# kieranrcampbell/clonealign

Measured on AMD Instinct MI355X. Metric: ELBO iterations/sec, higher is better.
Workload: dtype f32 variables (contraction: float64 series over gene bins; count-matrix products: int8 MFMA, exact); 1 GPU; synthetic 100000 cells x 5000 genes x 8 clones, K=1, S=1, cell-sharded over 1 GPU(s) (BASELINE.json configs[2]); cells=100000, genes=5000, clones=8, K=1, mc_samples=1, y_storage=u8, y_bytes_per_elem=1, fused_sweep=True, fwd_mfma=True, series_form=True, y_mfma=True, parallelism=single, collective=none, allreduce_doubles_per_train_pass=20764, build_id=cf8e5d62109b05e5

## Files before the change

### clonealign_amd/csrc/ca_eng_create.inc

```

constexpr double CA_ML_STREAM_FIXED_US = 6.6;
constexpr double CA_ML_STREAM_BYTES_PER_US = 5.62e6;
constexpr double CA_ML_MIN_STREAM_US = 45.0;
constexpr int CA_ML_MAX_PER = 4;
struct ca_mom_last_in {
  int slots;
  int n_cu;
  int nb_stream, nb_ovf;
  int ngrp, nred;
  int64_t image_bytes;
};
inline int ca_mom_last_free(const ca_mom_last_in& a) { return std::max(a.slots - a.nb_stream, 0); }
inline int ca_mom_last_free_x(const ca_mom_last_in& a) {
  const int xcd = std::max(a.n_cu / 32, 1);
  return a.slots / xcd - cdiv(a.nb_stream, xcd);
}
inline int ca_mom_last_per(const ca_mom_last_in& a) {
  const int xcd = std::max(a.n_cu / 32, 1), free_x = ca_mom_last_free_x(a);
  if (free_x < 1) return 0;
  return std::max(1, cdiv(a.ngrp, free_x * xcd));
}
inline bool ca_mom_last_pick(const ca_mom_last_in& a) {
  if (a.nb_stream + a.ngrp + a.nred <= a.slots) return false;
  const int per = ca_mom_last_per(a);
// ... 451 lines not shown
    h->mom_free_slots = ca_mom_last_free(ml);
    h->mom_last = variantx_on(h, CA_VARX_MOM_LAST, "CA_MOM_LAST_ON") || (variant_on(h, CA_VAR_MOM_LAST, "CA_MOM_LAST") && ca_mom_last_pick(ml));
    if (h->opt.variant_off & CA_VAR_MOM_LAST) h->mom_last = false;
    if (h->mom_last) {
      const int per = ca_mom_last_per(ml);
      h->mom_per = per < 1 ? CA_MOM_PER : std::min(per, CA_ML_MAX_PER);
      h->mom_nred = 2 * CA_MOM_NRED;
      const int lab = (h->opt.reserved[1] & ~0xFF) ? h->opt.reserved[1] >> 8 : 0;
      if (lab & 15) h->mom_per = lab & 15;
      if (lab & 16) h->mom_nred = CA_MOM_NRED;
      h->mom_ovf_first = (lab & 32) != 0;
    }
  }
  h->cell_lean = h->poly && variant_on(h, CA_VAR_CELL_LEAN, "CA_CELL_LEAN");
  h->cell_mfma = h->poly && variant_on(h, CA_VAR_CELL_MFMA, "CA_CELL_MFMA");
  h->gene_ride = h->poly && variant_on(h, CA_VAR_GENE_RIDE, "CA_GENE_RIDE");
  h->gene_cols = h->gene_ride && (h->opt.reserved[1] == 8 || (h->opt.reserved[1] != 7 && Nn <= CA_GENE_COLS_MAXN));
  h->ride_ok = h->ystore == CA_YSTORE_U8 && K == 1 && D <= 2 && h->fused_ok && !h->c16 && h->fwd_cell && (h->fc_tl == 6 || h->fc_tl == 8 || (h->fc_tl == 2 && h->fc_nbig == 0)) &&
               !h->y_ys && variant_on(h, CA_VAR_Y_RIDE, "CA_Y_RIDE");
  const bool tl1_ok = h->fc_tl == 1 && h->fc_nbig == 0 && !h->c16;
  h->ride_ys = h->y_ys && (!h->ys4 || (h->poly && D == 1 && !h->c16 && !h->s2)) && D <= 2 && h->fused_ok && h->fwd_cell && (h->fc_tl == 6 || tl1_ok || (h->fc_tl == 2 && h->fc_nbig == 0)) &&
               variant_on(h, CA_VAR_Y_RIDE, "CA_Y_RIDE");
  h->yfin_split = h->ride_ys && h->bwd_mfma && h->tail_fuse && variant_on(h, CA_VAR_YFIN_RIDE, "CA_YFIN_RIDE");
  if (h->y_ys && !h->ride_ys) h->async_y = false;
  {
    const int tiles = cdiv(Nn, 16), qb = tiles / std::max(h->n_cu, 1), rb = tiles - qb * h->n_cu;
    h->fwd_bal = h->ride_ys && !h->c16 && !h->s2 && D == 1 && C <= 8 && qb >= 1 && qb <= 6 && h->nk32 >= 96 && h->host_dev && variant_on(h, CA_VAR_FWD_BAL, "CA_FWD_BAL");
    if (h->fwd_bal) {
      h->bal_q = qb; h->bal_r = rb;
      h->bal_nchunk = rb > 0 ? std::min(CA_BAL_MAXCHUNK, h->n_cu / rb) : 0;
// ... 103 lines not shown
```

### clonealign_amd/csrc/ca_eng_loop.inc

```
int wait_y(ca_engine* h, bool all) {
  if (all) {
    if (h->y_pending) HIPCK(h, hipStreamWaitEvent(h->stream, h->ev_ydone, 0));
    h->y_pending = false; h->yw_pending = false;
  } else if (h->yw_pending) {
    HIPCK(h, hipStreamWaitEvent(h->stream, h->ev_ywdone, 0));
    h->yw_pending = false;
  }
  return CA_OK;
}

int make_etamax(ca_engine* h) {
  if (h->D > 0) {
    LAUNCH(h, CA_KERNEL_OTHER, hipLaunchKernelGGL(k_vmm_final, dim3(1), dim3(64), 0, h->stream, h->vmm_part, h->vmm, h->ngblk, h->D));
    LAUNCH(h, CA_KERNEL_OTHER, hipLaunchKernelGGL(k_etamax, dim3(cdiv(h->N, CA_TB)), dim3(CA_TB), 0, h->stream, h->F, h->vmm, h->etamax2, h->N, h->D));
  }
  h->em_stale = false;
  return CA_OK;
}
int ensure_etamax(ca_engine* h) {
  if (!h->em_stale) return CA_OK;
  return make_etamax(h);
}

int refresh_derived(ca_engine* h) {
// ... 758 lines not shown
    if (yfin_rides) { yfin_ride = yfin_args(h, h->ys_nrg, h->ys_nseg); h->yfin_pending = false; }
    if (moments_aside) HIPCK(h, hipStreamWaitEvent(h->stream, h->ev_poly1, 0));
    CACK(prof_begin(h, CA_KERNEL_FWD));
    ca_small_args ltail = no_small_args();
    const bool sh = is_sharded(h) && h->tail_fuse && yfin_rides;
    if (sh) {
      ltail = small_args(h, h->gene_part, 0, 0.f, nullptr, true);
      ltail.ncblk = h->pws.n_cell_blocks;
      if (h->K > 0) { ltail.yw_part = h->yw_part; ltail.n_yw = h->n_yw; }
      ltail.reduce_only = 1; ltail.host_out = nullptr;
    }
    const bool cols_move = yfin_rides && h->gene_cols;
    const bool merges = gene_ride_merges(h);
    ca_yfin_args yfin_cols = yfin_ride;
    if (cols_move) yfin_ride.ncol = 0;
    e = ca_poly_cells(h->stream, &h->pws, h->N, h->C, h->K, &cp, h->alpha_u, h->cell_part, h->dFpart, yfin_rides ? &yfin_ride : nullptr, h->cell_lean, h->cell_mfma);
    h->red_pending = merges;
    if (merges) h->ycol_pending = cols_move;
    else if (e == hipSuccess)
      e = ca_poly_reduce(h->stream, &h->pws, h->N, h->C, cols_move ? &yfin_cols : nullptr, sh ? &ltail : nullptr, h->poly_xmax_ready ? h->poly_xpart : nullptr,
                         (int)cdiv(h->N, CA_TB), h->F, sh ? h->red + h->off_x : nullptr, h->opt.rank, std::max(h->opt.world, 1));
    h->mon_tail_local = sh;
    if (sh) { h->poly_xslot_pending = true; h->poly_xglob_steps = -1; }
    HIPCK(h, e);
    CACK(prof_end(h));
    cell_blocks = h->pws.n_cell_blocks;
    h->poly_fresh = true;
  } else
  if (h->fwd_cell && ride && h->ride_ys) {
    cell_blocks = h->ncblk_f;
    CACK(ys_quant(h));
// ... 201 lines not shown
```

### clonealign_amd/csrc/ca_eng_state.inc

```
namespace {

thread_local std::string g_last_error;

typedef struct { char internal[128]; } ca_nccl_uid;
typedef void* ca_nccl_comm;
struct RcclApi {
  void* lib = nullptr;
  int (*GetUniqueId)(ca_nccl_uid*) = nullptr;
  int (*CommInitRank)(ca_nccl_comm*, int, ca_nccl_uid, int) = nullptr;
  int (*CommDestroy)(ca_nccl_comm) = nullptr;
  int (*AllReduce)(const void*, void*, size_t, int, int, ca_nccl_comm, hipStream_t) = nullptr;
  const char* (*GetErrorString)(int) = nullptr;
  std::string err;
  bool load() {
    if (lib) return true;
    const char* cands[] = {getenv("CLONEALIGN_RCCL_LIB"), "librccl.so.1", "librccl.so", "/opt/rocm/lib/librccl.so.1",
                           "/opt/rocm/lib/librccl.so"};
    for (const char* c : cands) {
      if (!c || !*c) continue;
      lib = dlopen(c, RTLD_NOW | RTLD_LOCAL);
      if (lib) break;
    }
    if (!lib) { err = std::string("cannot dlopen librccl: ") + dlerror(); return false; }
    GetUniqueId = (decltype(GetUniqueId))dlsym(lib, "ncclGetUniqueId");
// ... 103 lines not shown
  bool poly_shape = false, layout_series = false;
  bool mon_tail_local = false;
  bool poly_xslot_pending = false;
  int poly_xglob_steps = -1;
  double* elbo_dev = nullptr; int64_t elbo_cap = 0; double* terms_dev = nullptr;
  double* host_pinned = nullptr;
  bool ycache_valid = false, sums_global = false, sums_started = false;
  std::vector<double> mu_part;
  bool fused_ok = false, look_valid = false; int64_t look_slot = 0; int frow = 8;
  bool carry = false, carry_builtin = false; std::vector<float> carry_eps;
  int64_t n_series = 0, n_series_fallback = 0;
  double *poly_ring = nullptr, *poly_ring_dev = nullptr; uint64_t poly_seq = 0, poly_seq_base = 1, adam_steps = 0, poly_steps_at[16] = {};
  bool mom_ride = false; unsigned mom_tag = 0; const ca_pm_args* mom_args = nullptr;
  bool mom_last = false, mom_ovf_first = false; int mom_free_slots = 0, mom_per = CA_MOM_PER, mom_nred = CA_MOM_NRED;
  bool cell_mfma = false;
  bool cell_lean = false;
  bool gene_cols = false;
  bool gene_ride = false, red_pending = false, ycol_pending = false; unsigned gene_tag = 0; int poly_nb_ub = 0;
  bool poly = false, poly_side = false, poly_y_defer = false, poly_fresh = false, poly_df = false ; ca_poly_ws pws; float* poly_zero = nullptr; unsigned char* poly_mem = nullptr;
  float *Mb2 = nullptr, *mu32B = nullptr, *Zpart2 = nullptr; double* gene_partB = nullptr;
  bool y_defer = false;
  bool ride_ok = false;
  bool ride_ys = false;
  bool fold_gsum = false, fold_now = false;
  int64_t hint_A = -1, hint_B = -1, pre_A = -1, pre_B = -1;
  bool pre_valid = false, pre_ok = true, pair_elbo = true;
  double* ee_partB = nullptr;
  double *gene_part_alt = nullptr, *gene_partB_alt = nullptr;
  bool bwd_ready = false; int64_t bwd_slot = -1;
  double* yw_part = nullptr; int n_yw = 0;
// ... 53 lines not shown
  } while (0)

int comm_check(ca_engine* h) {
  if (h->host_pinned && *reinterpret_cast<volatile unsigned int*>(h->host_pinned + 41) != 0u) {
    h->err = "a forward-sweep block gave up waiting for a chunk of a left-over tile (k_fwd_bal_ys); the engine's state is undefined";
    return CA_ERR_STATE;
  }
  if (h->host_pinned && *reinterpret_cast<volatile unsigned int*>(h->host_pinned + 43) != 0u) {
    h->err = "a reducer block of the series form's moment role gave up waiting for the moment blocks of its launch (k_ys_mfma_mom); the engine's state is undefined";
    return CA_ERR_STATE;
  }
  if (h->host_pinned && *reinterpret_cast<volatile unsigned int*>(h->host_pinned + 44) != 0u) {
    h->err = "a gene block of the series form's merged way back gave up waiting for the reducer blocks of its launch (k_poly_tail); the engine's state is undefined";
    return CA_ERR_STATE;
  }
  if (h->host_pinned && *reinterpret_cast<volatile unsigned int*>(h->host_pinned + 42) != 0u) {
    h->err = "the series form of the contraction (CA_VARX_SERIES) cannot cover this fit's exponent range: max|psi| (max W - min W) exceeds 4 x " +
             std::to_string(CA_PL_NB) + " bins' worth; the passes since are truncated -- start over without the series form";
    return CA_ERR_STATE;
  }
  if (h->p2p && h->p2p->err_host && *reinterpret_cast<volatile unsigned long long*>(h->p2p->err_host) != 0ull) {
    h->err = "peer-to-peer all-reduce #" + std::to_string(*reinterpret_cast<volatile unsigned long long*>(h->p2p->err_host)) +
             ": a peer's data did not arrive within the time limit (peer lost or out of step); this engine's transport is dead -- "
             "destroy the engine and start over in a fresh process";
    return CA_ERR_COMM;
  }
  return CA_OK;
}
#define SYNC(h)                                          \
  do {                                                   \
// ... 291 lines not shown
```

### clonealign_amd/csrc/ca_poly.h

```cpp
#pragma once
#include <hip/hip_runtime.h>
#include <stddef.h>
#include <stdint.h>

#define CA_PL_R 20
#define CA_PL_NB 32
#define CA_PL_A 2.0
#ifndef CA_PL_NBL
#define CA_PL_NBL 4
#endif

struct ca_poly_hdr { double vlo, delta, xmax; int nb, bad; };
#define CA_PL_NGFLAG 256
struct ca_poly_ws {
  ca_poly_hdr* hdr; unsigned int* xbits; unsigned int* mflags ; unsigned int* gflags ; double *tabB, *partB, *tabQ, *Qpart;
  int n_cell_blocks, n_gene_blocks;
};

inline bool ca_poly_ok(int D, int S, int C) { return D == 1 && S == 1 && C >= 3 && C <= 8; }
size_t ca_poly_workspace_bytes(int G, int n_cell_blocks);
void ca_poly_bind(ca_poly_ws* w, void* base, int G, int n_cell_blocks);
hipError_t ca_poly_moments(hipStream_t st, const ca_poly_ws* w, const float* V, const float* F, const float* muA, const float* muB, const float* Lb, int G,
                           int64_t N, int C, unsigned int* bad_word ,
                           double* mirror , double seq, const float* xpart, int nx,
// ... 6 lines not shown
  return x * wdt / (2.0 * CA_PL_A);
}
inline bool ca_poly_covers(double xmax, double vlo, double vhi, int steps, double step_bound) {
  const double b = ca_poly_bins_ahead(xmax, vlo, vhi, steps, step_bound);
  return b == b && b <= (double)CA_PL_NB;
}
inline int ca_poly_nb_ahead(double xmax, double vlo, double vhi, int steps, double step_bound) {
  const double b = ca_poly_bins_ahead(xmax, vlo, vhi, steps, step_bound);
  if (!(b == b) || b > (double)CA_PL_NB) return 0;
  const int nb = (int)b + ((double)(int)b < b ? 1 : 0);
  return nb < 1 ? 1 : nb;
}
hipError_t ca_poly_cells(hipStream_t st, const ca_poly_ws* w, int64_t N, int C, int K, const void* cell_ptrs, const float* alpha_u, double* cell_part, float* dF,
                         const void* yfin_args ,
                         bool lean ,
                         bool mfma );
hipError_t ca_poly_reduce(hipStream_t st, const ca_poly_ws* w, int64_t N, int C,
                          const void* yfin_cols ,
                          const void* local_tail ,
                          const float* xs_part, int xs_n, const float* xs_F, double* xs_slots ,
                          int rank, int world);
hipError_t ca_poly_backward(hipStream_t st, const ca_poly_ws* w, const float* V, const float* mu, const float* Lb, int G, int C, double* red_g,
                            const void* small_tail );
hipError_t ca_poly_backward_merged(hipStream_t st, const ca_poly_ws* w, const float* V, const float* mu, const float* Lb, int G, int C, double* red_g,
                                   const void* small_tail, const void* yfin_cols ,
                                   int nb_hint ,
                                   unsigned int tag , unsigned long long timeout_ticks ,
                                   unsigned int* err );
```

### clonealign_amd/csrc/ca_poly.hip

```cpp
#include <hip/hip_runtime.h>
#include <stdint.h>

#include <algorithm>
#include <cstring>
#include <type_traits>

#include "ca_poly.h"

namespace ca_series {
#include "ca_kernels.hip.h"

constexpr int R = CA_PL_R, NB = CA_PL_NB;
#include "ca_polymom.hip.h"
constexpr int TB_B = 384;
constexpr int GPB = CA_PM_GPB;

__device__ __forceinline__ float warp_max(float v) {
#pragma unroll
  for (int o = 32; o > 0; o >>= 1) v = fmaxf(v, __shfl_xor(v, o, 64));
  return v;
}
__device__ __forceinline__ float warp_min(float v) {
#pragma unroll
  for (int o = 32; o > 0; o >>= 1) v = fminf(v, __shfl_xor(v, o, 64));
// ... 248 lines not shown
      for (int i = 0; i < 2; ++i)
#pragma unroll
        for (int j = 0; j < NCT; ++j)
#pragma unroll
          for (int r = 0; r < 4; ++r) {
            const int k = 16 * i + 4 * r + mk, col = j * 16 + mrow, b = j * BPT + mbl;
            if (k < RQ && b < nb && mcl < C) mine[(b * RQ + k) * C + mcl] = ((qm[i][j][r] + p1[k * (NBR * CP) + col]) + p2[k * (NBR * CP) + col]) + p3[k * (NBR * CP) + col];
          }
    }
  } else if (qown) {
#pragma unroll
    for (int b = 0; b < NBR; ++b) if (b < nb) mine[(b * RQ + qk) * C + qc] = qa[b];
  }
}

struct ca_xslot_args { const float* xpart; int nx; const float* F; int64_t N; double* slots; int rank, world; };
__device__ __forceinline__ void ca_poly_xslot_body(const ca_xslot_args& a) {
  __shared__ float sx[CA_TB / 64];
  float ax = 0.f;
  if (a.nx > 0) { for (int i = threadIdx.x; i < a.nx; i += CA_TB) ax = fmaxf(ax, a.xpart[i]); }
  else { for (int64_t i = threadIdx.x; i < a.N; i += CA_TB) { const float v = fabsf(a.F[i]); ax = fmaxf(ax, v == v ? v : INFINITY); } }
  ax = warp_max(ax);
  if ((threadIdx.x & 63) == 0) sx[threadIdx.x >> 6] = ax;
  __syncthreads();
  if ((int)threadIdx.x < a.world) a.slots[threadIdx.x] = (int)threadIdx.x == a.rank ? (double)fmaxf(fmaxf(sx[0], sx[1]), fmaxf(sx[2], sx[3])) : 0.0;
}
template <bool COLS>
__global__ void __launch_bounds__(CA_TB) k_poly_red(const double* __restrict__ part, int nblk, int64_t stride, const ca_poly_hdr* __restrict__ hdr, int per_bin,
                                                    int mode, int C, double* __restrict__ out, unsigned int* __restrict__ xbits, int nred, ca_small_args tail,
                                                    ca_xslot_args xs, int nfix, ca_yfin_args yfin) {
// ... 78 lines not shown
  memset(&a, 0, sizeof(a));
  a.V = V; a.xbits = w->xbits; a.muA = muA; a.muB = muB; a.Lb = Lb; a.G = G; a.C = C; a.hdr = w->hdr; a.part = w->partB; a.bad_word = bad_word; a.mirror = mirror; a.seq = seq;
  a.xpart = xpart; a.nx = nglob ? 0 : nx; a.xglob = xglob; a.nglob = nglob; a.xadd = xadd;
  hipLaunchKernelGGL(k_poly_B, dim3(w->n_gene_blocks), dim3(TB_B), 0, st, a);
  {
    ca_small_args no_tail; memset(&no_tail, 0, sizeof(no_tail));
    ca_xslot_args no_xs; memset(&no_xs, 0, sizeof(no_xs));
    ca_yfin_args no_yfin; memset(&no_yfin, 0, sizeof(no_yfin));
    hipLaunchKernelGGL(k_poly_red<false>, dim3(256), dim3(CA_TB), 0, st, w->partB, w->n_gene_blocks, (int64_t)NB * (R + 1) * 16, w->hdr,
                       (R + 1) * 16, 0, C, w->tabB, w->xbits, 256, no_tail, no_xs, 0, no_yfin);
  }
  return hipGetLastError();
}

hipError_t ca_poly_cells(hipStream_t st, const ca_poly_ws* w, int64_t N, int C, int K, const void* cell_ptrs, const float* alpha_u, double* cell_part, float* dF,
                         const void* yfin_args, bool lean, bool mfma) {
  const ca_cell_ptrs& p = *static_cast<const ca_cell_ptrs*>(cell_ptrs);
  ca_yfin_args yfin;
  if (yfin_args) memcpy(&yfin, yfin_args, sizeof(yfin)); else memset(&yfin, 0, sizeof(yfin));
  int CP = 1;
  while (CP < C) CP <<= 1;
  const int nextra = yfin_args ? cdiv_i(yfin.ncol, CA_TB / 64) + yfin.nrow : 0;
  const dim3 grid(w->n_cell_blocks + nextra);
#define CA_PCELL(CPV, LV) do { if (mfma) CA_PCELL_(CPV, LV, true); else CA_PCELL_(CPV, LV, false); } while (0)
#define CA_PCELL_(CPV, LV, MV) hipLaunchKernelGGL((k_poly_cell<CPV, LV, MV>), grid, dim3(CA_TB), 0, st, w->hdr, w->tabB, p, alpha_u, cell_part, N, C, K, dF, w->Qpart, \
                                         w->n_cell_blocks, yfin)
  if (lean) {
    if (K > 1) return hipErrorInvalidValue;
    if (CP == 4) CA_PCELL(4, true); else CA_PCELL(8, true);
  } else {
    if (CP == 4) CA_PCELL(4, false); else CA_PCELL(8, false);
  }
#undef CA_PCELL
#undef CA_PCELL_
  return hipGetLastError();
}

constexpr int NRED_Q = 256;
// ... 53 lines not shown
```

### clonealign_amd/csrc/clonealign_hip.hip

```cpp
#include "clonealign_hip.h"

#include <dlfcn.h>
#include <unistd.h>
#include <hip/hip_runtime.h>

#include <algorithm>
#include <cmath>
#include <cstdio>
#include <cstring>
#include <string>
#include <atomic>
#include <chrono>
#include <thread>
#include <vector>

#include "ca_kernels.hip.h"
#include "ca_poly.h"
#include "philox_host.h"

#include "ca_eng_state.inc"
#include "ca_eng_launch.inc"
#include "ca_eng_reduce.inc"
#include "ca_eng_loop.inc"
#include "ca_eng_ingest.inc"
// ... 310 lines not shown
  i->y_stream_bits = h->y_ys ? (h->ys4 ? 4 : 8) : 0;
  i->y_stream_n2 = h->ys_n2;
  i->y_stream_esc = h->ys_n2 > 0 ? h->n_esc2 : h->ys4 ? h->n_esc : 0;
  i->y_stream_bytes = !h->y_ys ? 0 : h->ys_n2 > 0 ? (h->ys_N64 / 64) * (int64_t)h->ys_nseg * (h->ys_n2 * 1024 + (8 - h->ys_n2) * 2048) + 4 * h->n_esc2
                                   : h->ys4 ? h->ys_N64 * h->Gp / 2 + 4 * h->n_esc : h->ys_N64 * h->Gp;
  i->y_ride = (h->ride_ok || h->ride_ys) ? 1 : 0;
  i->transport = (h->p2p && h->p2p->connected) ? CA_TRANSPORT_P2P : h->comm ? CA_TRANSPORT_RCCL : h->host_ar ? CA_TRANSPORT_HOST : CA_TRANSPORT_NONE;
  i->red_n = h->red_n;
  i->fwd_block_cells = (h->fused_ok && h->fwd_cell) ? 16 * h->fc_tl : 0; i->fwd_blocks_big = h->fc_nbig;
  i->fwd_balanced = h->fwd_bal ? h->bal_q : 0;
  i->fwd_series = h->poly ? 1 : 0; i->series_passes = h->n_series; i->series_fallbacks = h->n_series_fallback;
  i->mom_ride = h->mom_ride ? 1 : 0;
  i->cell_lean = h->cell_lean ? 1 : 0; i->cell_mfma = h->cell_mfma ? 1 : 0;
  i->mom_last = h->mom_last ? 1 : 0; i->mom_free_slots = h->mom_free_slots;
  i->gene_ride = gene_ride_merges(h) ? 1 : 0;
  i->fold_gsum = (h->fold_gsum && !is_sharded(h)) ? 1 : 0; i->yfin_split = (h->yfin_split && !is_sharded(h)) ? 1 : 0;
  i->update_merge = (h->upd_merge && h->fused_ok && h->fwd_cell && h->K > 0) ? 1 : 0;
  return CA_OK;
}

int ca_stream_busy(ca_handle h, int32_t* busy) {
  if (!h || !busy) return CA_ERR_INVALID;
  const hipError_t q = hipStreamQuery(h->stream);
  if (q != hipSuccess && q != hipErrorNotReady) HIPCK(h, q);
  *busy = q == hipErrorNotReady ? 1 : 0;
  if (q == hipErrorNotReady) (void)hipGetLastError();
  return CA_OK;
}

int ca_synchronize(ca_handle h) {
// ... 318 lines not shown
    for (int64_t c = 0; c < r.cols; ++c)
      buf[i * r.stride + r.off + c] = (float)in[r.matrix ? hidx(h->layout, i, c, r.rows, r.cols) : i];
  CACK(upload_f(h, r.f, buf));
  CACK(refresh_derived(h));
  SYNC(h);
  return CA_OK;
}

int ca_reinit(ca_handle h, const double* psi0, const double* loc0) {
  if (!h) return CA_ERR_INVALID;
  CA_NOT_IN_RUN(h);
  if (h->K > 0 && !psi0) { h->err = "psi0 is required when K > 0"; return CA_ERR_INVALID; }
  HIPCK(h, hipSetDevice(h->device));
  CACK(wait_y(h, true));
  HIPCK(h, hipStreamSynchronize(h->stream));
  if (h->host_pinned) { *reinterpret_cast<volatile unsigned int*>(h->host_pinned + 41) = 0u; *reinterpret_cast<volatile unsigned int*>(h->host_pinned + 42) = 0u; *reinterpret_cast<volatile unsigned int*>(h->host_pinned + 43) = 0u; *reinterpret_cast<volatile unsigned int*>(h->host_pinned + 44) = 0u; }
  SYNC(h);
  const int64_t N = h->N; const int G = h->G, C = h->C, K = h->K, D = h->D;
  auto zero = [&](float* p, int64_t n) { return p && n > 0 ? hipMemsetAsync(p, 0, (size_t)n * sizeof(float), h->stream) : hipSuccess; };
  const int64_t GD = (int64_t)G * std::max(D, 1), NK = N * std::max(K, 1);
  HIPCK(h, zero(h->V, GD)); HIPCK(h, zero(h->m_V, GD)); HIPCK(h, zero(h->v_V, GD));
  HIPCK(h, zero(h->ls, G)); HIPCK(h, zero(h->m_ls, G)); HIPCK(h, zero(h->v_ls, G));
  HIPCK(h, zero(h->m_loc, G)); HIPCK(h, zero(h->v_loc, G));
  HIPCK(h, zero(h->vchi, std::max(K, 1))); HIPCK(h, zero(h->m_v, std::max(K, 1))); HIPCK(h, zero(h->v_v, std::max(K, 1)));
  HIPCK(h, zero(h->alpha_u, C)); HIPCK(h, zero(h->m_a, C)); HIPCK(h, zero(h->v_a, C));
  HIPCK(h, zero(h->glogit, N * C)); HIPCK(h, zero(h->m_gl, N * C)); HIPCK(h, zero(h->v_gl, N * C));
  HIPCK(h, zero(h->m_psi, NK)); HIPCK(h, zero(h->v_psi, NK));
  if (loc0) {
    std::vector<float> l0((size_t)G);
    for (int g = 0; g < G; ++g) l0[g] = (float)loc0[g];
    CACK(upload_f(h, h->loc, l0));
// ... 129 lines not shown
```

### clonealign_amd/engine.py

```python
import ctypes as C
import os

import numpy as np

from . import hostprep

_HERE = os.path.dirname(os.path.abspath(__file__))
LIB_PATH = os.path.join(_HERE, "libclonealign_hip.so")

CA_OK = 0
CA_ERR_NAN = 4
CA_INTERRUPTED = 7
CA_ABI_VERSION = 6
P2P_HANDLE_BYTES = 128
CA_F64, CA_F32, CA_I32, CA_U16, CA_U8 = 0, 1, 2, 3, 4
CA_ROW_MAJOR, CA_COL_MAJOR = 0, 1
YSTORE = {"auto": 0, "f32": 1, "u16": 2, "u8": 3}
YSTORE_NAME = {v: k for k, v in YSTORE.items()}
KERNEL_NAMES = ("fwd", "bwd", "ypass", "cell", "other")
VARIANTS = {"fused": 1 << 0, "fwd_mfma": 1 << 1, "fwd_cell": 1 << 2, "bwd_mfma": 1 << 3, "tail_fuse": 1 << 4, "async_y": 1 << 5,
            "pre": 1 << 6, "pair_elbo": 1 << 7, "prep_fast": 1 << 8, "update_merge": 1 << 9, "p2p": 1 << 10, "fold_gsum": 1 << 11, "y_ride": 1 << 12, "ride_seq": 1 << 13, "y_mfma1": 1 << 14, "yfin_ride": 1 << 15, "p2p_ride": 1 << 16, "run_gate": 1 << 17, "s2_fuse": 1 << 18, "fwd_bal": 1 << 19, "bwd_tl3": 1 << 20, "series": 1 << 21, "y4": 1 << 22, "mom_ride": 1 << 23, "cell_lean": 1 << 24, "mom_last": 1 << 25, "cell_mfma": 1 << 26, "y2": 1 << 27, "gene_ride": 1 << 28}
VARIANTS_ON = {"y_mfma2": 1 << 0, "async_small": 1 << 1, "y_mfma1": 1 << 2, "fold_always": 1 << 3, "ride_seq": 1 << 4, "p2p_same_device": 1 << 5, "run_fwd": 1 << 6, "bal_tiles": 1 << 7, "series": 1 << 8, "y4": 1 << 9, "mom_last": 1 << 10, "y2": 1 << 11}
OPT_VERBOSE = 0x80000000
TUNE = {"gsplit": 0, "fsplit": 1, "fc_tl": 2, "fc_nbig": 3, "csplit": 4, "csplit_m": 5, "tr": 6, "rg": 7}
TRANSPORT_NAME = {0: "none", 1: "rccl", 2: "host", 3: "p2p"}

EXPORTS = (
    "ca_abi_version", "ca_build_id", "ca_device_count", "ca_default_options", "ca_create", "ca_destroy", "ca_last_error", "ca_get_info",
    "ca_synchronize", "ca_stream_busy", "ca_comm_unique_id", "ca_comm_init", "ca_p2p_export", "ca_p2p_connect", "ca_p2p_commit", "ca_comm_benchmark", "ca_comm_selftest", "ca_set_host_allreduce", "ca_gamma_init", "ca_elbo", "ca_elbo_terms",
    "ca_step", "ca_gradients", "ca_run", "ca_run_ex", "ca_iterate", "ca_final_elbo", "ca_init_psi_pca", "ca_clone_gene_sums", "ca_get_param", "ca_set_param",
    "ca_get_gradient", "ca_reinit", "ca_get_kernel_times", "ca_reset_kernel_times", "ca_set_profile", "ca_eps_draw", "ca_allele_loglik", "ca_preprocess",
    "ca_group_create", "ca_group_destroy", "ca_group_last_error", "ca_group_get_info", "ca_group_rank_handle", "ca_group_init_psi_pca", "ca_group_gamma_init",
    "ca_group_elbo", "ca_group_step", "ca_group_run_ex", "ca_group_iterate", "ca_group_final_elbo", "ca_group_get_param", "ca_group_reinit",
    "ca_group_clone_gene_sums",
    "ca_create_sparse", "ca_group_create_sparse",
    "ca_fit_mse", "ca_group_fit_mse",
# ... 46 lines not shown
                ("variant_off", C.c_uint32), ("tune", C.c_int32 * 8), ("variant_on", C.c_uint32),
                ("ride_pattern", C.c_int32), ("comm_timeout_ms", C.c_int32), ("gate_timeout_us", C.c_int32), ("reserved", C.c_int32 * 2)]


class CaInfo(C.Structure):
    _fields_ = [("N", C.c_int64), ("G", C.c_int32), ("C", C.c_int32), ("K", C.c_int32), ("P", C.c_int32),
                ("S", C.c_int32), ("y_storage", C.c_int32), ("y_bytes_per_elem", C.c_int32),
                ("y_device_bytes", C.c_int64), ("device_bytes", C.c_int64), ("gsplit", C.c_int32),
                ("csplit", C.c_int32), ("n_cu", C.c_int32), ("fused_sweep", C.c_int32), ("fwd_mfma", C.c_int32),
                ("bwd_mfma", C.c_int32), ("fsplit", C.c_int32), ("fwd_cell", C.c_int32), ("y_mfma", C.c_int32),
                ("transport", C.c_int32), ("y_ride", C.c_int32), ("red_n", C.c_int64),
                ("fwd_block_cells", C.c_int32), ("fwd_blocks_big", C.c_int32), ("fold_gsum", C.c_int32), ("yfin_split", C.c_int32),
                ("update_merge", C.c_int32), ("fwd_balanced", C.c_int32), ("fwd_series", C.c_int32), ("y_stream_bits", C.c_int32),
                ("series_passes", C.c_int64), ("series_fallbacks", C.c_int64), ("mom_ride", C.c_int32), ("cell_lean", C.c_int32),
                ("mom_last", C.c_int32), ("mom_free_slots", C.c_int32), ("cell_mfma", C.c_int32),
                ("y_stream_n2", C.c_int32), ("y_stream_esc", C.c_int64), ("y_stream_bytes", C.c_int64), ("gene_ride", C.c_int32)]


class CaGroupInfo(C.Structure):
    _fields_ = [("world", C.c_int32), ("transport", C.c_int32), ("p2p_status", C.c_int32), ("rccl_status", C.c_int32),
                ("rebuilds", C.c_int32), ("selftest_rounds", C.c_int32), ("N", C.c_int64), ("note", C.c_char * 384)]


class CaPreprocessParams(C.Structure):
    _fields_ = [("min_counts_per_gene", C.c_double), ("min_counts_per_cell", C.c_double),
                ("remove_outlying_genes", C.c_int32), ("remove_genes_same_copy_number", C.c_int32),
                ("nmads", C.c_double), ("max_copy_number", C.c_double)]


HOST_ALLREDUCE_FN = C.CFUNCTYPE(C.c_int, C.c_void_p, C.POINTER(C.c_double), C.c_int64)
POLL_FN = C.CFUNCTYPE(C.c_int, C.c_void_p, C.c_int32, C.c_double)
# ... 1082 lines not shown
```

### include/clonealign_hip.h

```cpp
#ifndef CLONEALIGN_HIP_H
#define CLONEALIGN_HIP_H

#include <stdint.h>

#ifdef __cplusplus
extern "C" {
#endif

#define CA_ABI_VERSION 6

typedef struct ca_engine* ca_handle;

enum ca_status {
  CA_OK = 0,
  CA_ERR_INVALID = 1,
  CA_ERR_HIP = 2,
  CA_ERR_NOMEM = 3,
  CA_ERR_NAN = 4,
  CA_ERR_COMM = 5,
  CA_ERR_STATE = 6,
  CA_INTERRUPTED = 7
};

enum ca_dtype { CA_F64 = 0, CA_F32 = 1, CA_I32 = 2, CA_U16 = 3, CA_U8 = 4 };
// ... 37 lines not shown
  CA_VAR_FWD_BAL = 1 << 19,
  CA_VAR_BWD_TL3 = 1 << 20,
  CA_VAR_SERIES = 1 << 21,
  CA_VAR_P2P = 1 << 10,
  CA_VAR_FOLD_GSUM = 1 << 11,
  CA_VAR_Y_RIDE = 1 << 12,
  CA_VAR_Y_MFMA1 = 1 << 14,
  CA_VAR_YFIN_RIDE = 1 << 15,
  CA_VAR_Y4 = 1 << 22,
  CA_VAR_MOM_RIDE = 1 << 23,
  CA_VAR_CELL_LEAN = 1 << 24,
  CA_VAR_MOM_LAST = 1 << 25,
  CA_VAR_CELL_MFMA = 1 << 26,
  CA_VAR_Y2 = 1 << 27,
  CA_VAR_GENE_RIDE = 1 << 28,
  CA_VAR_RIDE_SEQ = 1 << 13
};
enum ca_variant_on {
  CA_VARX_Y_MFMA2 = 1 << 0,
  CA_VARX_Y_MFMA1 = 1 << 2,
  CA_VARX_FOLD_ALWAYS = 1 << 3,
  CA_VARX_RIDE_SEQ = 1 << 4,
  CA_VARX_P2P_SAME_DEVICE = 1 << 5,
  CA_VARX_RUN_FWD = 1 << 6,
  CA_VARX_BAL_TILES = 1 << 7,
  CA_VARX_SERIES = 1 << 8,
  CA_VARX_Y4 = 1 << 9,
  CA_VARX_MOM_LAST = 1 << 10,
  CA_VARX_Y2 = 1 << 11,
  CA_VARX_ASYNC_SMALL = 1 << 1
// ... 46 lines not shown
  int32_t update_merge;
  int32_t fwd_balanced;
  int32_t fwd_series;
  int32_t y_stream_bits;
  int64_t series_passes;
  int64_t series_fallbacks;
  int32_t mom_ride;
  int32_t cell_lean;
  int32_t mom_last;
  int32_t mom_free_slots;
  int32_t cell_mfma;
  int32_t y_stream_n2;
  int64_t y_stream_esc;
  int64_t y_stream_bytes;
  int32_t gene_ride;
} ca_info;
enum ca_transport { CA_TRANSPORT_NONE = 0, CA_TRANSPORT_RCCL = 1, CA_TRANSPORT_HOST = 2, CA_TRANSPORT_P2P = 3 };

enum ca_kernel_id {
  CA_KERNEL_FWD = 0,
  CA_KERNEL_BWD = 1,
  CA_KERNEL_YPASS = 2,
  CA_KERNEL_CELL = 3,
  CA_KERNEL_OTHER = 4,
  CA_KERNEL_COUNT = 5
};

int ca_abi_version(void);
const char* ca_build_id(void);
int ca_device_count(int32_t* n);
// ... 223 lines not shown
```

Measured before the change: 10510 iterations/s.

## Add wide per-thread-clone cell kernel for series form with register-tiled bins

Adds k_poly_cell_wide, a series-form cell kernel in which each lane evaluates all clones of a cell as vectors, holds up to four bins in fixed register tiles, and accumulates the bin moments with f64 MFMA across several passes before a single block-level reduction. It is enabled by default (variant_on) when cell_lean, cell_mfma, K<=1 and a pinned host flag are available, and is used only when the bin count is between 1 and 4. The aim is to cut per-pass shared-memory traffic and reduction overhead in the cell stage. In exchange it adds a new error flag that the host polls, a hard limit on bins, and a second large kernel to maintain.

Result: no change. 10470 iterations/s (-0.5%).

```diff
diff --git a/clonealign_amd/csrc/ca_eng_create.inc b/clonealign_amd/csrc/ca_eng_create.inc
--- a/clonealign_amd/csrc/ca_eng_create.inc
+++ b/clonealign_amd/csrc/ca_eng_create.inc
@@ -489,6 +489,7 @@
   }
   h->cell_lean = h->poly && variant_on(h, CA_VAR_CELL_LEAN, "CA_CELL_LEAN");
   h->cell_mfma = h->poly && variant_on(h, CA_VAR_CELL_MFMA, "CA_CELL_MFMA");
+  h->cell_wide = h->cell_lean && h->cell_mfma && K <= 1 && h->host_dev && variant_on(h, CA_VAR_CELL_WIDE, "CA_CELL_WIDE");
   h->gene_ride = h->poly && variant_on(h, CA_VAR_GENE_RIDE, "CA_GENE_RIDE");
   h->gene_cols = h->gene_ride && (h->opt.reserved[1] == 8 || (h->opt.reserved[1] != 7 && Nn <= CA_GENE_COLS_MAXN));
   h->ride_ok = h->ystore == CA_YSTORE_U8 && K == 1 && D <= 2 && h->fused_ok && !h->c16 && h->fwd_cell && (h->fc_tl == 6 || h->fc_tl == 8 || (h->fc_tl == 2 && h->fc_nbig == 0)) &&
diff --git a/clonealign_amd/csrc/ca_eng_loop.inc b/clonealign_amd/csrc/ca_eng_loop.inc
--- a/clonealign_amd/csrc/ca_eng_loop.inc
+++ b/clonealign_amd/csrc/ca_eng_loop.inc
@@ -796,7 +796,10 @@
     const bool merges = gene_ride_merges(h);
     ca_yfin_args yfin_cols = yfin_ride;
     if (cols_move) yfin_ride.ncol = 0;
-    e = ca_poly_cells(h->stream, &h->pws, h->N, h->C, h->K, &cp, h->alpha_u, h->cell_part, h->dFpart, yfin_rides ? &yfin_ride : nullptr, h->cell_lean, h->cell_mfma);
+    const bool wide = h->cell_wide && !cp.s2 && h->poly_nb_ub >= 1 && h->poly_nb_ub <= 4;
+    if (wide) ++h->n_cell_wide;
+    e = ca_poly_cells(h->stream, &h->pws, h->N, h->C, h->K, &cp, h->alpha_u, h->cell_part, h->dFpart, yfin_rides ? &yfin_ride : nullptr, h->cell_lean, h->cell_mfma,
+                      wide ? reinterpret_cast<unsigned int*>(h->host_dev + 45) : nullptr);
     h->red_pending = merges;
     if (merges) h->ycol_pending = cols_move;
     else if (e == hipSuccess)
diff --git a/clonealign_amd/csrc/ca_eng_state.inc b/clonealign_amd/csrc/ca_eng_state.inc
--- a/clonealign_amd/csrc/ca_eng_state.inc
+++ b/clonealign_amd/csrc/ca_eng_state.inc
@@ -141,6 +141,7 @@
   bool mom_ride = false; unsigned mom_tag = 0; const ca_pm_args* mom_args = nullptr;
   bool mom_last = false, mom_ovf_first = false; int mom_free_slots = 0, mom_per = CA_MOM_PER, mom_nred = CA_MOM_NRED;
   bool cell_mfma = false;
+  bool cell_wide = false; int64_t n_cell_wide = 0;
   bool cell_lean = false;
   bool gene_cols = false;
   bool gene_ride = false, red_pending = false, ycol_pending = false; unsigned gene_tag = 0; int poly_nb_ub = 0;
@@ -224,6 +225,10 @@
     h->err = "a gene block of the series form's merged way back gave up waiting for the reducer blocks of its launch (k_poly_tail); the engine's state is undefined";
     return CA_ERR_STATE;
   }
+  if (h->host_pinned && *reinterpret_cast<volatile unsigned int*>(h->host_pinned + 45) != 0u) {
+    h->err = "the series form's wide cell launch met a header with more bins than its register tiles hold (k_poly_cell_wide); the engine's state is undefined";
+    return CA_ERR_STATE;
+  }
   if (h->host_pinned && *reinterpret_cast<volatile unsigned int*>(h->host_pinned + 42) != 0u) {
     h->err = "the series form of the contraction (CA_VARX_SERIES) cannot cover this fit's exponent range: max|psi| (max W - min W) exceeds 4 x " +
              std::to_string(CA_PL_NB) + " bins' worth; the passes since are truncated -- start over without the series form";
diff --git a/clonealign_amd/csrc/ca_poly.h b/clonealign_amd/csrc/ca_poly.h
--- a/clonealign_amd/csrc/ca_poly.h
+++ b/clonealign_amd/csrc/ca_poly.h
@@ -44,7 +44,8 @@
 hipError_t ca_poly_cells(hipStream_t st, const ca_poly_ws* w, int64_t N, int C, int K, const void* cell_ptrs, const float* alpha_u, double* cell_part, float* dF,
                          const void* yfin_args ,
                          bool lean ,
-                         bool mfma );
+                         bool mfma ,
+                         unsigned int* wide_err );
 hipError_t ca_poly_reduce(hipStream_t st, const ca_poly_ws* w, int64_t N, int C,
                           const void* yfin_cols ,
                           const void* local_tail ,
diff --git a/clonealign_amd/csrc/ca_poly.hip b/clonealign_amd/csrc/ca_poly.hip
--- a/clonealign_amd/csrc/ca_poly.hip
+++ b/clonealign_amd/csrc/ca_poly.hip
@@ -286,6 +286,266 @@
   }
 }
 
+template <int CP> using ca_wide_dv = __attribute__((ext_vector_type(CP))) double;
+template <int CP> using ca_wide_fv = __attribute__((ext_vector_type(CP))) float;
+template <int CP>
+__device__ __forceinline__ double ca_wide_tsum(ca_wide_dv<CP> v) {
+  if constexpr (CP == 8) return ((v[0] + v[4]) + (v[2] + v[6])) + ((v[1] + v[5]) + (v[3] + v[7]));
+  else return (v[0] + v[2]) + (v[1] + v[3]);
+}
+template <int CP>
+__device__ __forceinline__ double ca_wide_tmax(ca_wide_dv<CP> v) {
+  if constexpr (CP == 8) return fmax(fmax(fmax(v[0], v[4]), fmax(v[2], v[6])), fmax(fmax(v[1], v[5]), fmax(v[3], v[7])));
+  else return fmax(fmax(v[0], v[2]), fmax(v[1], v[3]));
+}
+__device__ __forceinline__ double ca_wide_fma_u(double a, double b, double t) {
+  double r;
+  asm("v_fma_f64 %0, %1, %2, %3" : "=v"(r) : "v"(a), "v"(b), "s"(t));
+  return r;
+}
+__device__ __forceinline__ void ca_wide_acc_pass(ca_cell_acc& acc, bool okn, bool ok, int c, int K, double gam, double llpA, double llpB, double lg, double lac,
+                                                 double cn, double x) {
+  const bool live = ok && gam != 0.0;
+  if (ok) { acc.ee += gam * llpA; acc.pr += gam * lac; acc.eeB += gam * llpB; }
+  if (live) acc.q += gam * lg;
+  acc.gsumc += gam;
+  if (okn && c == 0) {
+    acc.ee += cn;
+    acc.eeB += cn;
+    if (K > 0) acc.pr += -0.5 * x * x - 0.5 * CA_LOG2PI;
+  }
+}
+template <int CP>
+__global__ void __launch_bounds__(CA_TB, 2) k_poly_cell_wide(const ca_poly_hdr* __restrict__ hdr, const double* __restrict__ tabB, ca_cell_ptrs p,
+                                                          const float* __restrict__ alpha_u, double* __restrict__ cell_part, int64_t N, int C, int K,
+                                                          float* __restrict__ dF , double* __restrict__ Qpart , int ncb, ca_yfin_args yfin,
+                                                          unsigned int* __restrict__ err) {
+  if ((int)blockIdx.x >= ncb) {
+    const int e = (int)blockIdx.x - ncb;
+    const int ncolblk = (yfin.ncol + CA_TB / 64 - 1) / (CA_TB / 64);
+    if (e < ncolblk) {
+      const int job = e * (CA_TB / 64) + (int)(threadIdx.x >> 6);
+      if (job < yfin.ncol) ca_yfin_col_wave(yfin, job);
+    } else if (e - ncolblk < yfin.nrow) {
+      __shared__ double ca_yfin_sm[CA_TB / 64];
+      ca_yfin_row_block(yfin, e - ncolblk, ca_yfin_sm);
+    }
+    return;
+  }
+  constexpr int CPB = CA_TB / CP;
+  constexpr int RQ = R + 2;
+  constexpr int NBR = 4;
+  constexpr int GW = 64 / CP;
+  constexpr int XSW = RQ + 1;
+  constexpr int O_V = 64 * NBR, O_CF = O_V + 64 * XSW, W_GATHER = 64 * XSW + 64 * CP / 2;
+  constexpr int O_PK = O_V, W_PARK = 4 * 64 * CP + 2 * 64;
+  constexpr int WSZ = O_V + (W_GATHER > W_PARK ? W_GATHER : W_PARK);
+  constexpr int QW = RQ * NBR * CP;
+  static_assert(WSZ >= QW, "a wave's tiles fit a wave's rows");
+  static_assert(CP == 4 || CP == 8, "the MFMA gather's column map");
+  static_assert(CA_TB == 256, "four waves");
+  __shared__ double sm[CA_TB];
+  __shared__ double la[64];
+  __shared__ double wl[CA_TB / 64][WSZ];
+  const int nb = hdr->nb;
+  if (nb > NBR) {
+    if (threadIdx.x == 0) { *reinterpret_cast<volatile unsigned int*>(err) = 1u; __threadfence_system(); }
+    return;
+  }
+  ca_log_softmax_alpha(alpha_u, C, la);
+  __syncthreads();
+  const int t = threadIdx.x, wv = t >> 6, l = t & 63;
+  const int lp = l / GW, slot = wv * GW + l % GW;
+  const int tc = t % CP, tslot = t / CP, tsrc = l / CP;
+  const double vlo = hdr->vlo, delta = hdr->delta;
+  double* const wme = wl[wv];
+  double* const w_xp = wme + O_V + l * XSW;
+  double* const w_eb = wme + l * NBR;
+  float* const w_cf = reinterpret_cast<float*>(wme + O_CF) + l * CP;
+  using qtile_t = __attribute__((ext_vector_type(4))) double;
+  constexpr int BPT = 16 / CP, NCT = NBR / BPT, KST = GW / 4;
+  qtile_t qm[2][NCT];
+#pragma unroll
+  for (int j = 0; j < NCT; ++j) { qm[0][j] = qtile_t{0.0, 0.0, 0.0, 0.0}; qm[1][j] = qtile_t{0.0, 0.0, 0.0, 0.0}; }
+  const int mrow = t & 15, mk = (t >> 4) & 3;
+  const int mcl = mrow % CP, mbl = mrow / CP;
+  double* mine = Qpart + (int64_t)blockIdx.x * (NB * RQ * 8);
+  ca_cell_acc acc = {0.0, 0.0, 0.0, 0.0, 0.0};
+  const int64_t ngroups = (N + CPB - 1) / CPB;
+  const int npass = (int64_t)blockIdx.x < ngroups ? (int)((ngroups - 1 - blockIdx.x) / ncb) + 1 : 0;
+  const double lac = la[tc < C ? tc : C - 1];
+  for (int sp0 = 0; sp0 < npass; sp0 += CP) {
+    const int np = npass - sp0 < CP ? npass - sp0 : CP;
+    const int64_t n = ((int64_t)blockIdx.x + (int64_t)(sp0 + lp) * ncb) * CPB + slot;
+    const bool okn = lp < np && n < N;
+    const int64_t nn = okn ? n : N - 1;
+    const double x = (double)p.F[nn];
+    const double sn = p.s64[nn], cn = p.cn[nn];
+    using dv = ca_wide_dv<CP>;
+    using fv = ca_wide_fv<CP>;
+    fv glf;
+#pragma unroll
+    for (int c = 0; c < CP; ++c) glf[c] = (okn && c < C) ? p.glogit[nn * C + (c < C ? c : C - 1)] : -INFINITY;
+    dv ZA, ZB, dZB;
+#pragma unroll
+    for (int c = 0; c < CP; ++c) { ZA[c] = 0.0; ZB[c] = 0.0; dZB[c] = 0.0; }
+#pragma unroll
+    for (int b = 0; b < NBR; ++b) w_eb[b] = 0.0;
+    for (int b = 0; b < nb; ++b) {
+      const double vb = vlo + ((double)b + 0.5) * delta;
+      const double e = exp(x * vb);
+      const double* __restrict__ tb = tabB + ((int64_t)b * (R + 1)) * 16;
+      dv pa, pb, dpb;
+#pragma unroll
+      for (int c = 0; c < CP; ++c) { pa[c] = tb[R * 16 + c]; pb[c] = tb[R * 16 + 8 + c]; dpb[c] = 0.0; }
+#pragma unroll 4
+      for (int k = R - 1; k >= 0; --k) {
+#pragma unroll
+        for (int c = 0; c < CP; ++c) {
+          dpb[c] = dpb[c] * x + pb[c];
+          pa[c] = ca_wide_fma_u(pa[c], x, tb[k * 16 + c]);
+          pb[c] = ca_wide_fma_u(pb[c], x, tb[k * 16 + 8 + c]);
+        }
+      }
+#pragma unroll
+      for (int c = 0; c < CP; ++c) { ZA[c] += e * pa[c]; ZB[c] += e * pb[c]; dZB[c] += e * (vb * pb[c] + dpb[c]); }
+      w_eb[b] = e;
+    }
+    dv Anc;
+#pragma unroll
+    for (int c = 0; c < CP; ++c) Anc[c] = p.A[nn * C + (c < C ? c : C - 1)];
+    dv gl;
+#pragma unroll
+    for (int c = 0; c < CP; ++c) gl[c] = (double)glf[c];
+    const double mx = ca_wide_tmax<CP>(gl);
+    dv ex;
+#pragma unroll
+    for (int c = 0; c < CP; ++c) ex[c] = (okn && c < C) ? exp(gl[c] - mx) : 0.0;
+    const double se = ca_wide_tsum<CP>(ex);
+    const double lse = mx + log(se);
+    dv gam, llpA, llpB, lg, fB, gfB, dfc;
+    fv cfo;
+    unsigned lv = 0u;
+#pragma unroll
+    for (int c = 0; c < CP; ++c) {
+      gam[c] = 0.0; llpA[c] = 0.0; llpB[c] = 0.0; lg[c] = 0.0; fB[c] = 0.0; gfB[c] = 0.0; cfo[c] = 0.f;
+      if (c < C) {
+        const bool ok = okn;
+        lg[c] = gl[c] - lse;
+        gam[c] = ok ? ex[c] / se : 0.0;
+        const double em = 0.0;
+        llpA[c] = Anc[c] - sn * (log(ZA[c]) + em);
+        llpB[c] = Anc[c] - sn * (log(ZB[c]) + em);
+        if (ok) cfo[c] = (float)(-gam[c] * sn / ZB[c]);
+        fB[c] = llpB[c] + la[c] - lg[c];
+        const bool live = ok && gam[c] != 0.0;
+        gfB[c] = (live || (ok && !isfinite(llpB[c]))) ? gam[c] * fB[c] : 0.0;
+        if (ok && (live || !isfinite(llpB[c]))) lv |= 1u << c;
+      }
+    }
+    const double fbarB = ca_wide_tsum<CP>(gfB);
+    fv dgo;
+#pragma unroll
+    for (int c = 0; c < CP; ++c) dgo[c] = (float)((lv >> c) & 1u ? gam[c] * (fB[c] - fbarB) : 0.0);
+    double dzl = dZB[0];
+#pragma unroll
+    for (int c = 1; c < CP; ++c) dzl = (c == C - 1) ? dZB[c] : dzl;
+#pragma unroll
+    for (int c = 0; c < CP; ++c) dfc[c] = (double)cfo[c] * (c < C ? dZB[c] : dzl);
+    const double df = ca_wide_tsum<CP>(dfc);
+    if (okn) {
+      dF[n] = (float)df;
+      if (C == CP) {
+        using f4 = __attribute__((ext_vector_type(4))) float;
+#pragma unroll
+        for (int q = 0; q < CP / 4; ++q) {
+          *reinterpret_cast<f4*>(p.coef + nn * CA_CW + 4 * q) = f4{cfo[4 * q], cfo[4 * q + 1], cfo[4 * q + 2], cfo[4 * q + 3]};
+          *reinterpret_cast<f4*>(p.dgl + nn * CP + 4 * q) = f4{dgo[4 * q], dgo[4 * q + 1], dgo[4 * q + 2], dgo[4 * q + 3]};
+        }
+      } else {
+#pragma unroll
+        for (int c = 0; c < CP; ++c) if (c < C) { p.coef[nn * CA_CW + c] = cfo[c]; p.dgl[nn * C + c] = dgo[c]; }
+      }
+      if (p.coefq) {
+#pragma unroll
+        for (int c = 0; c < CP; ++c) if (c < C) {
+          unsigned short p1, p2, p3;
+          ca_split3(cfo[c], p1, p2, p3);
+          unsigned short* qp = p.coefq + (nn * 4) * 8 + c;
+          qp[0] = p1; qp[8] = p2; qp[16] = p3;
+        }
+      }
+    }
+#pragma unroll
+    for (int c = 0; c < CP; ++c) {
+      wme[O_PK + (0 * 64 + l) * CP + c] = gam[c]; wme[O_PK + (1 * 64 + l) * CP + c] = llpA[c]; wme[O_PK + (2 * 64 + l) * CP + c] = llpB[c];
+      wme[O_PK + (3 * 64 + l) * CP + c] = lg[c];
+    }
+    wme[O_PK + 4 * 64 * CP + l] = cn; wme[O_PK + 4 * 64 * CP + 64 + l] = x;
+    __builtin_amdgcn_fence(__ATOMIC_RELEASE, "wavefront"); __builtin_amdgcn_wave_barrier(); __builtin_amdgcn_fence(__ATOMIC_ACQUIRE, "wavefront");
+    for (int pp = 0; pp < np; ++pp) {
+      const int src = pp * GW + tsrc;
+      const int64_t n_ = ((int64_t)blockIdx.x + (int64_t)(sp0 + pp) * ncb) * CPB + tslot;
+      const bool okn_ = n_ < N;
+      ca_wide_acc_pass(acc, okn_, okn_ && tc < C, tc, K, wme[O_PK + (0 * 64 + src) * CP + tc], wme[O_PK + (1 * 64 + src) * CP + tc],
+                       wme[O_PK + (2 * 64 + src) * CP + tc], wme[O_PK + (3 * 64 + src) * CP + tc], lac, wme[O_PK + 4 * 64 * CP + src],
+                       wme[O_PK + 4 * 64 * CP + 64 + src]);
+    }
+    __builtin_amdgcn_fence(__ATOMIC_RELEASE, "wavefront"); __builtin_amdgcn_wave_barrier(); __builtin_amdgcn_fence(__ATOMIC_ACQUIRE, "wavefront");
+    {
+      double xk = 1.0;
+#pragma unroll
+      for (int k = 0; k < RQ; ++k) { w_xp[k] = xk; xk *= x; }
+    }
+#pragma unroll
+    for (int c = 0; c < CP; ++c) w_cf[c] = cfo[c];
+    __builtin_amdgcn_fence(__ATOMIC_RELEASE, "wavefront"); __builtin_amdgcn_wave_barrier(); __builtin_amdgcn_fence(__ATOMIC_ACQUIRE, "wavefront");
+    for (int pp = 0; pp < np; ++pp) {
+#pragma unroll
+      for (int s = 0; s < KST; ++s) {
+        const int cl = pp * GW + s * 4 + mk;
+        const double a0 = wme[O_V + cl * XSW + mrow];
+        const double a1 = wme[O_V + cl * XSW + (16 + mrow < RQ ? 16 + mrow : RQ - 1)];
+        const double cfv = (double)reinterpret_cast<const float*>(wme + O_CF)[cl * CP + mcl];
+#pragma unroll
+        for (int j = 0; j < NCT; ++j) {
+          if (j == 0 || nb > j * BPT) {
+            const double bv = cfv * wme[cl * NBR + j * BPT + mbl];
+            qm[0][j] = __builtin_amdgcn_mfma_f64_16x16x4f64(a0, bv, qm[0][j], 0, 0, 0);
+            qm[1][j] = __builtin_amdgcn_mfma_f64_16x16x4f64(a1, bv, qm[1][j], 0, 0, 0);
+          }
+        }
+      }
+    }
+    __builtin_amdgcn_fence(__ATOMIC_RELEASE, "wavefront"); __builtin_amdgcn_wave_barrier(); __builtin_amdgcn_fence(__ATOMIC_ACQUIRE, "wavefront");
+  }
+  ca_cell_fused_finish<CP>(acc, sm, cell_part, blockIdx.x, C);
+  {
+    double* const p1 = wl[1], * const p2 = wl[2], * const p3 = wl[3];
+#pragma unroll
+    for (int i = 0; i < 2; ++i)
+#pragma unroll
+      for (int j = 0; j < NCT; ++j)
+#pragma unroll
+        for (int r = 0; r < 4; ++r) {
+          const int k = 16 * i + 4 * r + mk;
+          if (wv > 0 && k < RQ) wme[k * (NBR * CP) + j * 16 + mrow] = qm[i][j][r];
+        }
+    __syncthreads();
+    if (wv == 0) {
+#pragma unroll
+      for (int i = 0; i < 2; ++i)
+#pragma unroll
+        for (int j = 0; j < NCT; ++j)
+#pragma unroll
+          for (int r = 0; r < 4; ++r) {
+            const int k = 16 * i + 4 * r + mk, col = j * 16 + mrow, b = j * BPT + mbl;
+            if (k < RQ && b < nb && mcl < C) mine[(b * RQ + k) * C + mcl] = ((qm[i][j][r] + p1[k * (NBR * CP) + col]) + p2[k * (NBR * CP) + col]) + p3[k * (NBR * CP) + col];
+          }
+    }
+  }
+}
+
 struct ca_xslot_args { const float* xpart; int nx; const float* F; int64_t N; double* slots; int rank, world; };
 __device__ __forceinline__ void ca_poly_xslot_body(const ca_xslot_args& a) {
   __shared__ float sx[CA_TB / 64];
@@ -394,7 +654,7 @@
 }
 
 hipError_t ca_poly_cells(hipStream_t st, const ca_poly_ws* w, int64_t N, int C, int K, const void* cell_ptrs, const float* alpha_u, double* cell_part, float* dF,
-                         const void* yfin_args, bool lean, bool mfma) {
+                         const void* yfin_args, bool lean, bool mfma, unsigned int* wide_err) {
   const ca_cell_ptrs& p = *static_cast<const ca_cell_ptrs*>(cell_ptrs);
   ca_yfin_args yfin;
   if (yfin_args) memcpy(&yfin, yfin_args, sizeof(yfin)); else memset(&yfin, 0, sizeof(yfin));
@@ -402,6 +662,12 @@
   while (CP < C) CP <<= 1;
   const int nextra = yfin_args ? cdiv_i(yfin.ncol, CA_TB / 64) + yfin.nrow : 0;
   const dim3 grid(w->n_cell_blocks + nextra);
+  if (wide_err) {
+    if (!lean || !mfma || K > 1 || p.s2 || C < 3 || C > 8) return hipErrorInvalidValue;
+    if (CP == 4) hipLaunchKernelGGL(k_poly_cell_wide<4>, grid, dim3(CA_TB), 0, st, w->hdr, w->tabB, p, alpha_u, cell_part, N, C, K, dF, w->Qpart, w->n_cell_blocks, yfin, wide_err);
+    else hipLaunchKernelGGL(k_poly_cell_wide<8>, grid, dim3(CA_TB), 0, st, w->hdr, w->tabB, p, alpha_u, cell_part, N, C, K, dF, w->Qpart, w->n_cell_blocks, yfin, wide_err);
+    return hipGetLastError();
+  }
 #define CA_PCELL(CPV, LV) do { if (mfma) CA_PCELL_(CPV, LV, true); else CA_PCELL_(CPV, LV, false); } while (0)
 #define CA_PCELL_(CPV, LV, MV) hipLaunchKernelGGL((k_poly_cell<CPV, LV, MV>), grid, dim3(CA_TB), 0, st, w->hdr, w->tabB, p, alpha_u, cell_part, N, C, K, dF, w->Qpart, \
                                          w->n_cell_blocks, yfin)
diff --git a/clonealign_amd/csrc/clonealign_hip.hip b/clonealign_amd/csrc/clonealign_hip.hip
--- a/clonealign_amd/csrc/clonealign_hip.hip
+++ b/clonealign_amd/csrc/clonealign_hip.hip
@@ -348,6 +348,7 @@
   i->cell_lean = h->cell_lean ? 1 : 0; i->cell_mfma = h->cell_mfma ? 1 : 0;
   i->mom_last = h->mom_last ? 1 : 0; i->mom_free_slots = h->mom_free_slots;
   i->gene_ride = gene_ride_merges(h) ? 1 : 0;
+  i->cell_wide = h->cell_wide ? 1 : 0; i->cell_wide_passes = h->n_cell_wide;
   i->fold_gsum = (h->fold_gsum && !is_sharded(h)) ? 1 : 0; i->yfin_split = (h->yfin_split && !is_sharded(h)) ? 1 : 0;
   i->update_merge = (h->upd_merge && h->fused_ok && h->fwd_cell && h->K > 0) ? 1 : 0;
   return CA_OK;
@@ -696,7 +697,7 @@
   HIPCK(h, hipSetDevice(h->device));
   CACK(wait_y(h, true));
   HIPCK(h, hipStreamSynchronize(h->stream));
-  if (h->host_pinned) { *reinterpret_cast<volatile unsigned int*>(h->host_pinned + 41) = 0u; *reinterpret_cast<volatile unsigned int*>(h->host_pinned + 42) = 0u; *reinterpret_cast<volatile unsigned int*>(h->host_pinned + 43) = 0u; *reinterpret_cast<volatile unsigned int*>(h->host_pinned + 44) = 0u; }
+  if (h->host_pinned) { *reinterpret_cast<volatile unsigned int*>(h->host_pinned + 41) = 0u; *reinterpret_cast<volatile unsigned int*>(h->host_pinned + 42) = 0u; *reinterpret_cast<volatile unsigned int*>(h->host_pinned + 43) = 0u; *reinterpret_cast<volatile unsigned int*>(h->host_pinned + 44) = 0u; *reinterpret_cast<volatile unsigned int*>(h->host_pinned + 45) = 0u; }
   SYNC(h);
   const int64_t N = h->N; const int G = h->G, C = h->C, K = h->K, D = h->D;
   auto zero = [&](float* p, int64_t n) { return p && n > 0 ? hipMemsetAsync(p, 0, (size_t)n * sizeof(float), h->stream) : hipSuccess; };
diff --git a/clonealign_amd/engine.py b/clonealign_amd/engine.py
--- a/clonealign_amd/engine.py
+++ b/clonealign_amd/engine.py
@@ -19,7 +19,7 @@
 YSTORE_NAME = {v: k for k, v in YSTORE.items()}
 KERNEL_NAMES = ("fwd", "bwd", "ypass", "cell", "other")
 VARIANTS = {"fused": 1 << 0, "fwd_mfma": 1 << 1, "fwd_cell": 1 << 2, "bwd_mfma": 1 << 3, "tail_fuse": 1 << 4, "async_y": 1 << 5,
-            "pre": 1 << 6, "pair_elbo": 1 << 7, "prep_fast": 1 << 8, "update_merge": 1 << 9, "p2p": 1 << 10, "fold_gsum": 1 << 11, "y_ride": 1 << 12, "ride_seq": 1 << 13, "y_mfma1": 1 << 14, "yfin_ride": 1 << 15, "p2p_ride": 1 << 16, "run_gate": 1 << 17, "s2_fuse": 1 << 18, "fwd_bal": 1 << 19, "bwd_tl3": 1 << 20, "series": 1 << 21, "y4": 1 << 22, "mom_ride": 1 << 23, "cell_lean": 1 << 24, "mom_last": 1 << 25, "cell_mfma": 1 << 26, "y2": 1 << 27, "gene_ride": 1 << 28}
+            "pre": 1 << 6, "pair_elbo": 1 << 7, "prep_fast": 1 << 8, "update_merge": 1 << 9, "p2p": 1 << 10, "fold_gsum": 1 << 11, "y_ride": 1 << 12, "ride_seq": 1 << 13, "y_mfma1": 1 << 14, "yfin_ride": 1 << 15, "p2p_ride": 1 << 16, "run_gate": 1 << 17, "s2_fuse": 1 << 18, "fwd_bal": 1 << 19, "bwd_tl3": 1 << 20, "series": 1 << 21, "y4": 1 << 22, "mom_ride": 1 << 23, "cell_lean": 1 << 24, "mom_last": 1 << 25, "cell_mfma": 1 << 26, "y2": 1 << 27, "gene_ride": 1 << 28, "cell_wide": 1 << 29}
 VARIANTS_ON = {"y_mfma2": 1 << 0, "async_small": 1 << 1, "y_mfma1": 1 << 2, "fold_always": 1 << 3, "ride_seq": 1 << 4, "p2p_same_device": 1 << 5, "run_fwd": 1 << 6, "bal_tiles": 1 << 7, "series": 1 << 8, "y4": 1 << 9, "mom_last": 1 << 10, "y2": 1 << 11}
 OPT_VERBOSE = 0x80000000
 TUNE = {"gsplit": 0, "fsplit": 1, "fc_tl": 2, "fc_nbig": 3, "csplit": 4, "csplit_m": 5, "tr": 6, "rg": 7}
@@ -96,7 +96,8 @@
                 ("update_merge", C.c_int32), ("fwd_balanced", C.c_int32), ("fwd_series", C.c_int32), ("y_stream_bits", C.c_int32),
                 ("series_passes", C.c_int64), ("series_fallbacks", C.c_int64), ("mom_ride", C.c_int32), ("cell_lean", C.c_int32),
                 ("mom_last", C.c_int32), ("mom_free_slots", C.c_int32), ("cell_mfma", C.c_int32),
-                ("y_stream_n2", C.c_int32), ("y_stream_esc", C.c_int64), ("y_stream_bytes", C.c_int64), ("gene_ride", C.c_int32)]
+                ("y_stream_n2", C.c_int32), ("y_stream_esc", C.c_int64), ("y_stream_bytes", C.c_int64), ("gene_ride", C.c_int32),
+                ("cell_wide", C.c_int32), ("cell_wide_passes", C.c_int64)]
 
 
 class CaGroupInfo(C.Structure):
diff --git a/include/clonealign_hip.h b/include/clonealign_hip.h
--- a/include/clonealign_hip.h
+++ b/include/clonealign_hip.h
@@ -75,6 +75,7 @@
   CA_VAR_CELL_MFMA = 1 << 26,
   CA_VAR_Y2 = 1 << 27,
   CA_VAR_GENE_RIDE = 1 << 28,
+  CA_VAR_CELL_WIDE = 1 << 29,
   CA_VAR_RIDE_SEQ = 1 << 13
 };
 enum ca_variant_on {
@@ -151,6 +152,8 @@
   int64_t y_stream_esc;
   int64_t y_stream_bytes;
   int32_t gene_ride;
+  int32_t cell_wide;
+  int64_t cell_wide_passes;
 } ca_info;
 enum ca_transport { CA_TRANSPORT_NONE = 0, CA_TRANSPORT_RCCL = 1, CA_TRANSPORT_HOST = 2, CA_TRANSPORT_P2P = 3 };
 
```
